# ChenWu98/cycle-diffusion

Measured on AMD Instinct MI355X. Metric: images/sec, SD-v1.4 512px CycleDiffusion 100+100 steps, 1/2/4/8 MI355X, higher is better.
Workload: dtype fp16; 1 GPU; C2: Stable-Diffusion-v1.4-shaped U-Net + KL-f8 VAE, 512x512, custom_steps=99 white_box_steps=100 eta=0.1 skip 0, 1 trial, encoder scale 1, decoder CFG 3; batch_per_gpu=4, global_batch=4, parallelism=dp1, steps_per_launch_set=5, launch_set_cap=16, launch_sets_in_flight_per_gpu=1, images_in_flight_per_gpu=20, distributed=single process, weights=synthetic(seed=0)

## Files before the change

cycle-diffusion_amd/_ffi.py:

```python
import ctypes as C
import os

import numpy as np

_HERE = os.path.dirname(os.path.abspath(__file__))
LIB_PATH = os.path.join(_HERE, "lib", "libcyclediff.so")

CD_NET_UNET_OPENAI, CD_NET_UNET_HO, CD_NET_VAE_KL, CD_NET_CLIP_TEXT, CD_NET_BERT_XTR = 1, 2, 3, 4, 5
CD_NET_OCLIP_TEXT, CD_NET_OCLIP_VISION, CD_NET_INCEPTION_FID = 6, 7, 8
CD_SCHED_DDIM, CD_SCHED_DDPM = 0, 1
CD_PREC_16, CD_PREC_F32, CD_PREC_F32X3 = 0, 1, 2
CD_MASK_QSAMPLE, CD_MASK_ENCODER = 0, 1
MASK_SOURCES = {"q_sample": CD_MASK_QSAMPLE, "encoder": CD_MASK_ENCODER}
ACT_NONE, ACT_SILU, ACT_GELU, ACT_GEGLU, ACT_QGELU, ACT_RELU = 0, 1, 2, 3, 4, 5


class NetDesc(C.Structure):
    _fields_ = [
        ("kind", C.c_int), ("image_size", C.c_int), ("in_channels", C.c_int), ("out_channels", C.c_int),
        ("model_channels", C.c_int), ("num_res_blocks", C.c_int),
        ("n_mult", C.c_int), ("channel_mult", C.c_int * 8),
        ("n_attn", C.c_int), ("attn", C.c_int * 8),
        ("num_heads", C.c_int), ("num_head_channels", C.c_int),
        ("use_spatial_transformer", C.c_int), ("context_dim", C.c_int), ("transformer_depth", C.c_int),
# ... 46 lines not shown
    "cd_cycle_translate_masked": [_VP, _I, _I, _VP, _VP, _VP, _F, _VP, _VP, _F, _VP, _I, _I, _I, _I, _VP, _VP, _VP, _U64, _I,
                                  _VP, _VP, _I, _I, _VP, _VP, _U64, _VP, _VP],
    "cd_cycle_translate_ctrl": [_VP, _I, _I, _VP, _VP, _VP, _F, _VP, _VP, _F, _VP, _I, _I, _I, _I, _VP, _VP, _VP, _U64, _I,
                                _VP, _VP, _I, _I, _VP, _VP, _U64, _VP, _VP, _VP, _I, _I, _VP, _VP],
    "cd_pix_refine": [_VP, _I, _I, _VP, _I, _I, _VP, _VP, _U64],
    "cd_op_pack_conv_weight": [_VP, _VP, _I, _I, _I, _I, _I, C.POINTER(_VP), C.POINTER(_I), C.POINTER(_I)],
    "cd_op_free": [_VP, _VP],
    "cd_op_conv2d": [_VP, _VP, _I, _VP, _I, _I, _I, _I, _VP, _I, _I, _I, _I, _I, _I, _I, _VP, _VP, _VP, _I, _I, _VP],
    "cd_op_conv2d_16": [_VP, _VP, _I, _VP, _I, _I, _I, _I, _VP, _I, _I, _I, _I, _I, _I, _I, _VP, _VP, _VP, _I, _I, _VP,
                        _VP],
    "cd_op_last_gemm_config": [_VP] + [C.POINTER(_I)] * 5,
    "cd_op_up_phase_reorder": [_VP, _VP, _I, _I, _I, _I, _VP],
    "cd_op_groupnorm": [_VP, _VP, _I, _I, _I, _I, _I, _F, _VP, _VP, _VP, _I, _VP],
    "cd_op_groupnorm_ex": [_VP, _VP, _I, _I, _VP, _I, _I, _I, _I, _I, _F, _VP, _VP, _VP, _I, _I, _VP, _VP, _I, _VP],
    "cd_op_layernorm": [_VP, _VP, _I, _I, _VP, _VP, _F, _VP],
    "cd_op_attention": [_VP, _VP, _VP, _VP, _I, _I, _I, _I, _I, _F, _I, _VP],
    "cd_op_cross_attention_ctrl": [_VP, _VP, _VP, _VP, _VP, _VP, _VP, _VP, _VP, _I, _I, _I, _I, _I, _I, _I, _I, _F, _VP],
    "cd_op_softmax_rows": [_VP, _VP, _I64, _I, _VP],
    "cd_op_timestep_embedding": [_VP, _VP, _I, _I, _I, _VP],
    "cd_op_sched_step": [_VP, _I, _I, _VP, _VP, _VP, _VP, _I, _F, _VP, _VP, _I, _I, _I, _I, _VP],
    "cd_op_sched_step_masked": [_VP, _I, _VP, _VP, _VP, _I, _F, _VP, _VP, _VP, _I, _I, _F, _F, _VP, _I, _I, _I, _I, _VP, _I],
    "cd_op_bench_conv": [_VP, _I, _I, _I, _I, _I, _I, _I, _I, _I, _I, _I, _I, C.POINTER(C.c_float)],
    "cd_op_bench_mfma_sustained": [_VP, _I, C.POINTER(C.c_float), C.POINTER(C.c_float)],
    "cd_op_probe": [_VP, _I, _VP, _VP, _SZ],
}
_RESTYPES = {"cd_last_error": C.c_char_p}

_lib = None


# ... 45 lines not shown
```

cycle-diffusion_amd/csrc/capi.hip:

```cpp
#include <stdlib.h>
#include <string.h>
#include <unistd.h>

#include <algorithm>

#include "engine.h"

using namespace cd;

struct StepPacer {
  static constexpr int kAhead = 2, kRing = kAhead + 1;
  hipEvent_t ev[kRing] = {nullptr, nullptr, nullptr};
  long n = 0;
  bool enabled = true;
  void init() {
    const char* e = getenv("CYCLEDIFF_HOST_PACING");
    enabled = !(e && e[0] == '0');
    for (auto& x : ev) HIP_CHECK(hipEventCreateWithFlags(&x, hipEventBlockingSync | hipEventDisableTiming));
  }
  static void sleep_until_done(hipEvent_t e) {
    for (;;) {
      const hipError_t q = hipEventQuery(e);
      if (q == hipSuccess) return;
      if (q != hipErrorNotReady) HIP_CHECK(q);
// ... 1087 lines not shown

int cd_op_layernorm(cd_handle h, const float* x, int rows, int C, const float* gamma, const float* beta,
                    float eps, float* y) {
  CD_API_BEGIN
  enter_engine(h);
  CD_CHECK(h && x && y, "bad argument");
  ArenaScope arena_scope(h->arena);
  bf16_t* a = (bf16_t*)h->arena.alloc((size_t)rows * C * 2);
  bf16_t* o = (bf16_t*)h->arena.alloc((size_t)rows * C * 2);
  launch_nchw_to_nhwc(h->st, x, a, rows, C, 1, C, 1.f, 0.f, 0);
  launch_layernorm(h->st, a, C, o, C, rows, C, gamma, beta, eps);
  launch_nhwc_to_nchw(h->st, o, 0, C, y, rows, C, 1, 1.f, 0.f);
  CD_API_END
}

int cd_op_attention(cd_handle h, const float* q, const float* k, const float* v, int B, int H, int Tq,
                    int Tk, int D, float scale, int use_transpose_kernel, float* o) {
  CD_API_BEGIN
  enter_engine(h);
  CD_CHECK(h && q && k && v && o, "bad argument");
  ArenaScope arena_scope(h->arena);
  const int C = H * D, Tpad = round_up(Tk, 64);
  bf16_t* qb = (bf16_t*)h->arena.alloc((size_t)B * Tq * C * 2);
  bf16_t* kb = (bf16_t*)h->arena.alloc((size_t)B * Tk * C * 2);
  bf16_t* vb = (bf16_t*)h->arena.alloc((size_t)B * Tk * C * 2);
  bf16_t* ob = (bf16_t*)h->arena.alloc((size_t)B * Tq * C * 2);
  launch_nchw_to_nhwc(h->st, q, qb, B * Tq, C, 1, C, 1.f, 0.f, 0);
  launch_nchw_to_nhwc(h->st, k, kb, B * Tk, C, 1, C, 1.f, 0.f, 0);
  launch_nchw_to_nhwc(h->st, v, vb, B * Tk, C, 1, C, 1.f, 0.f, 0);
  AttnParams p;
// ... 297 lines not shown
```

cycle-diffusion_amd/csrc/conv_gemm.hip:

```cpp
#include <stdio.h>
#include <stdlib.h>
#include <string.h>

#include <algorithm>
#include <map>
#include <mutex>
#include <string>

#include "common.h"
#include "kernels.h"

namespace cd {

namespace gemm_detail {

#ifndef CD_EPI_STORE_AUX
#define CD_EPI_STORE_AUX 0
#endif
#ifndef CD_EPI_RESID_AUX
#define CD_EPI_RESID_AUX 0
#endif

typedef const __attribute__((address_space(1))) void* gptr_t;
typedef __attribute__((address_space(3))) void* lptr_t;
// ... 1170 lines not shown
void launch_conv_gemm(hipStream_t st, const ConvGemmParams& p) {
  const int Ctot = p.C0 + p.C1;
  CD_CHECK(p.C0 % 32 == 0 && p.C1 % 32 == 0, "conv_gemm: channels must be multiples of 32 (C0=%d C1=%d)", p.C0, p.C1);
  CD_CHECK(p.Ktot == p.KH * p.KW * Ctot, "conv_gemm: Ktot mismatch");
  CD_CHECK(p.zeros != nullptr, "conv_gemm: zero page missing");
  CD_CHECK(p.M > 0 && p.N > 0, "conv_gemm: empty problem");
  CD_CHECK(((uintptr_t)p.src0 & 15) == 0 && ((uintptr_t)p.wgt & 15) == 0, "conv_gemm: 16-B alignment");
  CD_CHECK((p.ld0 % 8) == 0 && (p.src1 == nullptr || (p.ld1 % 8) == 0), "conv_gemm: ld must be a multiple of 8");
  if (p.act == ACT_GEGLU) CD_CHECK(p.N % 64 == 0, "GEGLU needs packed N %% 64 == 0");
  if (p.up_phase)
    CD_CHECK(p.KH == 2 && p.KW == 2 && p.stride == 1 && !p.up && !p.src1 && p.nbatch == 1 && p.Hout == p.Hs && p.Wout == p.Ws &&
                 (p.Hs * p.Ws) % 256 == 0 && p.M == 4 * p.B * p.Hs * p.Ws && p.w_ps > 0 && p.Hin == p.Hs && p.Win == p.Ws,
             "conv_gemm: phase form of an x2 conv on %d x %d", p.Hs, p.Ws);
  bool k64 = (p.C0 % 64 == 0) && (p.C1 % 64 == 0);
  if (p.ln_fold) CD_CHECK(p.tile == kLinStreamTile, "conv_gemm: a LayerNorm-folded layer runs on lin_stream only");
  int id = p.tile ? p.tile : tuned_config(st, p, k64);
  if (id & (1 << 16)) k64 = false;
  ConvGemmParams pk = p;
  id &= 0xffff;
  if ((id >> 8) > 1) pk.splitk = id >> 8;
  id &= 0xff;
  if (pk.splitk > 1 && !pk.sk_scratch) { pk.sk_scratch = g_conv_splitk.scratch; pk.sk_flags = g_conv_splitk.flags; }
  pk.probe = g_conv_probe;
  static const int korder_env = [] { const char* e = getenv("CYCLEDIFF_KORDER"); return e ? atoi(e) : -1; }();
  if (korder_env >= 0) pk.korder = korder_env;
  static const int tg_env = [] { const char* e = getenv("CYCLEDIFF_TILE_GROUP"); return e ? atoi(e) : 8; }();
  static const int tg_min_n = [] { const char* e = getenv("CYCLEDIFF_TILE_GROUP_MIN_N"); return e ? atoi(e) : 2048; }();
  if (tg_env > 0 && p.N >= tg_min_n && p.nbatch == 1) pk.tile_group = tg_env;
#ifdef CD_PROBE
  if (const char* e = getenv("CYCLEDIFF_PROBE_DBG")) pk.dbg = atoi(e);
// ... 117 lines not shown
```

cycle-diffusion_amd/csrc/engine.h:

```cpp
#pragma once
#include <map>
#include <memory>
#include <string>
#include <vector>

#include "common.h"
#include "kernels.h"
#include "../../include/cyclediff.h"

namespace cd {

class Arena {
 public:
  ~Arena();
  void init(size_t bytes);
  void* alloc(size_t bytes);
  size_t mark() const { return off_; }
  void release(size_t m) { off_ = m; }
  void reset() { off_ = 0; }
  size_t capacity() const { return cap_; }
  size_t high_water() const { return high_; }
 private:
  char* base_ = nullptr;
  size_t cap_ = 0, off_ = 0, high_ = 0;
// ... 93 lines not shown

struct ConvOpts {
  int stride = 1;
  int pad = 1;
  bool asym = false;
  bool up = false;
  const float* rowvec = nullptr; int rowvec_ld = 0; int rows_per_vec = 1;
  const Act* resid = nullptr;
  int act = ACT_NONE;
  float alpha = 1.f;
  bool out_f32 = false;
  void* out = nullptr;
  int out_ld = 0;
  bool ln_fold = false;
  float ln_eps = 1e-5f;
  bool raw_geglu = false;
  bool want_stats = false;
  float* out_stats = nullptr;
  int tile = 0;
};
Act attention_flash_f32_fwd(Ctx& c, const float* q, int ldq, const float* k, int ldk, int64_t k_bs, const float* v, int ldv,
                            int64_t v_bs, int B, int H, int Tq, int Tk, int D, float scale, int Himg, int Wimg, bool q_log2);
Act geglu_f32_fwd(Ctx& c, const Act& h);
Act split_rows_f32_fwd(Ctx& c, const Act& x, const Act* x2 = nullptr);
Act alloc_act(Ctx& c, int B, int H, int W, int C, bool with_stats = false);
Act conv_fwd(Ctx& c, const ConvW& w, const Act& x, const Act* x2, const ConvOpts& o);
bool conv_up_phase_taken(const Ctx& c, const ConvW& w, const Act& x, const Act* x2, const ConvOpts& o);
bool conv_ln_fold_available(const Ctx& c, const ConvW& w, int64_t rows);

struct GNW { float* g = nullptr; float* b = nullptr; int C = 0; float eps = 1e-5f; };
Act groupnorm_fwd(Ctx& c, const GNW& w, const Act& x, const Act* x2, bool silu, const float* film = nullptr,
                  int film_ld = 0);
struct LNW { float* g = nullptr; float* b = nullptr; int C = 0; };
Act layernorm_fwd(Ctx& c, const LNW& w, const Act& x);

Act avgpool2_fwd(Ctx& c, const Act& x);
Act upsample2_fwd(Ctx& c, const Act& x);
Act attention_f32_fwd(Ctx& c, const Act& qk, const Act& v, int H, int D, float scale, const float* obias);

Act attention_fwd(Ctx& c, const bf16_t* q, int ldq, const bf16_t* k, int ldk, const bf16_t* v, int ldv, int B,
                  int H, int Tq, int Tk, int D, float scale, int Himg, int Wimg, bool q_log2 = false);
Act attention_vt_fwd(Ctx& c, const bf16_t* q, int ldq, const bf16_t* k, int ldk, const bf16_t* vt, int B,
                     int H, int Tq, int Tk, int Tpad, int D, float scale, int Himg, int Wimg, bool q_log2 = false);
// ... 80 lines not shown
```

cycle-diffusion_amd/csrc/engine.hip:

```cpp
#include <stdlib.h>

#include "engine.h"

#include <string.h>

namespace cd {

Arena::~Arena() { if (base_) (void)hipFree(base_); }
void Arena::init(size_t bytes) {
  if (base_) { (void)hipFree(base_); base_ = nullptr; }
  HIP_CHECK(hipMalloc((void**)&base_, bytes));
  cap_ = bytes; off_ = 0; high_ = 0;
}
void* Arena::alloc(size_t bytes) {
  size_t a = (off_ + 255) & ~(size_t)255;
  CD_CHECK(a + bytes <= cap_, "workspace arena exhausted: need %zu more bytes (capacity %zu); "
           "create the engine with a larger workspace", a + bytes - cap_, cap_);
  off_ = a + bytes;
  if (off_ > high_) high_ = off_;
  return base_ + a;
}

ParamStore::~ParamStore() {
  for (void* p : allocs_) (void)hipFree(p);
// ... 309 lines not shown
  p.B = x.B; p.Hs = x.H; p.Ws = x.W; p.up = o.up ? 1 : 0;
  p.Hin = o.up ? x.H * 2 : x.H; p.Win = o.up ? x.W * 2 : x.W;
  p.KH = w.KH; p.KW = w.KW; p.stride = o.stride;
  if (o.asym) { p.pad_t = 0; p.pad_l = 0; p.Hout = (p.Hin + 1 - w.KH) / o.stride + 1; p.Wout = (p.Win + 1 - w.KW) / o.stride + 1; }
  else {
    p.pad_t = o.pad; p.pad_l = o.pad;
    p.Hout = (p.Hin + 2 * o.pad - w.KH) / o.stride + 1;
    p.Wout = (p.Win + 2 * o.pad - w.KW) / o.stride + 1;
  }
  p.M = x.B * p.Hout * p.Wout;
  p.wgt = w.w; p.wgt_frag = w.wfrag; p.Ktot = w.Ktot(); p.N = w.N;
  p.alpha = o.alpha; p.bias = w.b;
  p.rowvec = o.rowvec; p.rowvec_ld = o.rowvec_ld; p.rows_per_vec = o.rows_per_vec;
  const bool fuse_geglu = w.geglu && !o.raw_geglu;
  p.act = fuse_geglu ? ACT_GEGLU : o.act;
  const int Nout = fuse_geglu ? w.N / 2 : w.N;
  Act y; y.B = x.B; y.H = p.Hout; y.W = p.Wout; y.C = Nout; y.f32 = c.f32;
  if (o.out) { y.p = (bf16_t*)o.out; y.ld = o.out_ld; }
  else {
    y.ld = Nout;
    y.p = (bf16_t*)c.arena->alloc((size_t)p.M * Nout * ((o.out_f32 || c.f32) ? 4 : 2));
  }
  if (o.resid) {
    CD_CHECK(o.resid->rows() == p.M && o.resid->C == Nout, "conv: residual shape mismatch");
    p.resid = o.resid->p; p.resid_ld = o.resid->ld;
  }
  p.out = y.p; p.out_ld = y.ld; p.out_f32 = o.out_f32 ? 1 : 0;
  p.zeros = c.zeros; p.tile = o.tile;
  if (o.ln_fold) { p.ln_fold = 1; p.ln_eps = o.ln_eps; p.tile = kLinStreamTile; }
  if (c.f32) {
    p.out_f32 = 1;
    launch_conv_gemm_f32(c.st, p);
    return y;
  }
  if (!w.geglu && !o.out_f32 && ((p.Hout * p.Wout) % 32) == 0) {
    if (o.out && o.out_stats) y.stats_buf = o.out_stats;
    else if (!o.out && o.want_stats)
      y.stats_buf = (float*)c.arena->alloc((size_t)(p.M / 32) * 2 * Nout * sizeof(float));
    p.stats = y.stats_buf;
    y.stats = y.stats_buf;
  }
  launch_conv_gemm(c.st, p);
  return y;
}

bool conv_ln_fold_available(const Ctx& c, const ConvW& w, int64_t rows) {
  static const bool on = [] { const char* e = getenv("CYCLEDIFF_LN_FOLD"); return !(e && e[0] == '0'); }();
  static const int64_t min_rows = [] { const char* e = getenv("CYCLEDIFF_LN_FOLD_MIN_ROWS"); return e ? atoll(e) : 32768ll; }();
  return on && !c.f32 && w.wfrag && w.KH == 1 && w.KW == 1 && w.Cpad == 320 && rows >= min_rows && rows % 32 == 0 &&
         w.N % 64 == 0 && w.N <= 2560;
}

Act groupnorm_fwd(Ctx& c, const GNW& w, const Act& x, const Act* x2, bool silu, const float* film,
                  int film_ld) {
  GroupNormParams p;
  p.x = x.p; p.C0 = x.C; p.ld0 = x.ld;
  if (x2) { p.x1 = x2->p; p.C1 = x2->C; p.ld1 = x2->ld; }
  const int C = p.C0 + p.C1;
  CD_CHECK(C == w.C, "groupnorm: channels %d != weight %d", C, w.C);
  p.B = x.B; p.HW = x.H * x.W; p.G = 32; p.eps = w.eps; p.gamma = w.g; p.beta = w.b;
  p.film = film; p.film_ld = film_ld; p.silu = silu ? 1 : 0;
  Act y = alloc_act(c, x.B, x.H, x.W, C);
  p.y = y.p;
  if (c.f32) {
    CD_CHECK(x.f32 && (!x2 || x2->f32) && !x.split && (!x2 || !x2->split), "groupnorm: operand precision");
// ... 133 lines not shown
```

cycle-diffusion_amd/csrc/kernels.h:

```cpp
#pragma once
#include <map>
#include <string>
#include <vector>

#include "common.h"

namespace cd {

struct StepCoef {
  float sa, s1a, sap, dirc, sigma, r, t_mask;
  int t;
};
enum { SCHED_DDIM = 0, SCHED_DDPM = 1 };

struct EpsHat {
  const float* p = nullptr;
  int64_t sb = 0, sc = 0, sp = 0;
  int cfg = 0;
  float g = 1.f;
  const float* gvec = nullptr;
};

struct StepGeom {
  int B = 0, C = 0, HW = 0;
// ... 67 lines not shown
  float alpha = 1.0f;
  const float* bias = nullptr;
  const float* rowvec = nullptr;
  int rowvec_ld = 0, rows_per_vec = 1;
  const bf16_t* resid = nullptr;
  int resid_ld = 0;
  int resid_f32 = 0;
  int act = ACT_NONE;
  void* out = nullptr;
  int out_ld = 0;
  int out_f32 = 0;
  float* stats = nullptr;
  const bf16_t* zeros = nullptr;
  int ln_fold = 0;
  float ln_eps = 1e-5f;
  int tile = 0;
  float prof_flop_scale = 1.f;
  int splitk = 0;
  float* sk_scratch = nullptr;
  int* sk_flags = nullptr;
  unsigned long long* probe = nullptr;
  int korder = 1;
  int tile_group = 0;
  int dephase_ticks = 0;
  int num_cus = 256;
  int dbg = 0;
  int up_phase = 0;
  int w_ps = 0;
};
constexpr int kProbeWords = 48;
// ... 17 lines not shown
GemmLaunchInfo conv_gemm_last_launch();
void launch_up_phase_weights(hipStream_t st, const bf16_t* w, bf16_t* out, int Npad, int Cpad);
int conv_gemm_num_configs();
const char* conv_gemm_config_name(int id);

struct LinStreamParams {
  const bf16_t* a = nullptr; int lda = 0;
  const bf16_t* wfrag = nullptr;
  const float* bias = nullptr;
  const bf16_t* resid = nullptr; int ldr = 0;
  bf16_t* out = nullptr; int ldo = 0;
  float* stats = nullptr;
  int M = 0, N = 0;
  float ln_eps = 1e-5f;
  int geglu_direct = 0;
};
constexpr int kLinStreamTile = 30;
bool lin_stream_supports(const ConvGemmParams& p);
void launch_lin_stream(hipStream_t st, const ConvGemmParams& p);
void launch_fold_ln(hipStream_t st, const bf16_t* w, int ldw, const float* gamma, const float* beta, const float* bias,
                    bf16_t* w_out, float* bias_out, int N, int Kc);
void launch_pack_wfrag(hipStream_t st, const bf16_t* w, int ldw, bf16_t* out, int N);

struct KernelProfiler {
  bool enabled = false;
  std::vector<hipEvent_t> events;
  std::vector<double> flops;
  std::vector<std::string> labels;
  int used = 0;
  bool verbose = false;
// ... 136 lines not shown
```

cycle-diffusion_amd/csrc/lin_stream.hip:

```cpp
#include <stdlib.h>

#include <mutex>

#include "common.h"
#include "kernels.h"

namespace cd {
namespace lin_detail {

typedef __attribute__((address_space(3))) void* lptr_t;
typedef __attribute__((ext_vector_type(4))) unsigned int u32x4;

constexpr int K = 320, NKS = K / 16, KSH = NKS / 2;
constexpr int WPIECE = 2 * KSH * 1024, WSLOTS = 3;
constexpr int APIECE = 128 * 128, ASLOTS = 3;
constexpr int NAP = 10;
constexpr int ST_LD = 36, ST_BYTES = 32 * ST_LD * 4;
constexpr int BIAS_MAX = 2560;
constexpr int OFF_A = WSLOTS * WPIECE, OFF_ST = OFF_A + ASLOTS * APIECE, OFF_BIAS = OFF_ST + 8 * ST_BYTES;
constexpr int LDS_BYTES = OFF_BIAS + BIAS_MAX * 4;
static_assert(LDS_BYTES <= 160 * 1024, "LDS");
constexpr unsigned kNoLoad = 0x80000000u;
constexpr int kGegluDirectDefault = 1;

// ... 31 lines not shown
#pragma unroll
  for (int i = 0; i < 4; ++i) {
    const h2 v = {(_Float16)__builtin_amdgcn_fmed3f(f[2 * i], -65504.0f, 65504.0f),
                  (_Float16)__builtin_amdgcn_fmed3f(f[2 * i + 1], -65504.0f, 65504.0f)};
    w[i] = __builtin_bit_cast(uint32_t, v);
  }
  return make_uint4(w[0], w[1], w[2], w[3]);
#else
  return pack8(f);
#endif
}
__device__ __forceinline__ void touch4(u32x4& a, u32x4& b, u32x4& c, u32x4& d) {
  asm volatile("" : "+v"(a), "+v"(b), "+v"(c), "+v"(d)::"memory");
}

template <int ACT, bool RESID, bool STATS, bool LNF = false>
__global__ __launch_bounds__(512, 2) void k_lin_stream(LinStreamParams p) {
#if defined(__HIP_DEVICE_COMPILE__)
  constexpr bool GEGLU = (ACT == ACT_GEGLU);
  static_assert(!(GEGLU && (RESID || STATS)), "GEGLU has neither residual nor statistics");
  extern __shared__ __attribute__((aligned(16))) char smem[];
  char* wring = smem;
  char* aring = smem + OFF_A;
  const int tid = threadIdx.x, lane = tid & 63;
  const int wave = __builtin_amdgcn_readfirstlane(tid >> 6);
  float* stage = (float*)(smem + OFF_ST + wave * ST_BYTES);
  float* bias_s = (float*)(smem + OFF_BIAS);
  const int mi = lane & 31, half = lane >> 5;
  const bool w_issuer = wave < 4;
  const int wq = wave & 3;

  const int NT = p.N >> 6;
  const int I = 2 * NT;
  const int nstrips = (p.M + 255) >> 8;
  const int G = gridDim.x;
// ... 159 lines not shown
        const int soff = ((row0 + 16 * ps) * p.ldr + t * 64 + nb * 32) * 2;
        asm volatile("buffer_load_dwordx4 %0, %1, %2, %3 offen"
                     : "=v"(rres[nb * 2 + ps]) : "v"(r_lane), "s"(rs_r), "s"(soff) : "memory");
      }
    seq += 4;
    rmark = seq;
  };
  issue_resid((int)blockIdx.x * 256, 0);

  int gi = 0;
  int wslot = 0;
  for (int ord = 0; ord < my_count; ++ord) {
    const int row0 = ((int)blockIdx.x + ord * G) * 256;
    const bool has_next = ord + 1 < my_count;
    const bool rows_ok = row0 + wave * 32 < p.M;
    for (int t = 0; t < NT; ++t) {
#pragma unroll
      for (int r = 0; r < 16; ++r) { acc[0][r] = 0.f; acc[1][r] = 0.f; }
#pragma unroll
      for (int kh = 0; kh < 2; ++kh) {
        const int i = 2 * t + kh;
        if (w_issuer) wait_vmcnt_le(seq - wm0);
        const bool due = a_due(gi);
        if (due && !w_issuer) wait_vmcnt_le(seq - am0);
        asm volatile("s_waitcnt lgkmcnt(0)\n\ts_barrier" ::: "memory");
        if (w_issuer) {
          const int nxt = i + 2;
          const int slot2 = wslot == 0 ? 2 : wslot - 1;
          issue_w(nxt < I ? nxt : nxt - I, nxt < I || has_next, slot2);
          seq += 5;
          wm0 = wm1; wm1 = seq;
// ... 29 lines not shown
          }
        }
        if (due) take_a(ce_j, ce_slot);
        wslot = wslot == 2 ? 0 : wslot + 1;
        ++gi;
      }
      if (RESID && rows_ok) {
        wait_vmcnt_le(seq - rmark);
        touch4(rres[0], rres[1], rres[2], rres[3]);
      }
      float vv[2][8];
      int l2 = lane;
      asm volatile("" : "+v"(l2));
      const int prow = l2 >> 2, pcol = (l2 & 3) * 8, mi2 = l2 & 31, half2 = l2 >> 5;
      const unsigned o_lane = (unsigned)(((wave * 32 + prow) * p.ldo + pcol) * 2);
      if (GEGLU && p.geglu_direct) {
        const unsigned od_lane = (unsigned)(((wave * 32 + mi2) * p.ldo + 4 * half2) * 2);
#pragma unroll
        for (int q = 0; q < 4; ++q) {
          const float* bp = bias_s + t * 64 + 8 * q + 4 * half2;
          const f32x4 bv = *(const f32x4*)bp, bg = *(const f32x4*)(bp + 32);
          float val[4], gate[4], o4[4];
#pragma unroll
          for (int j = 0; j < 4; ++j) { val[j] = acc[0][4 * q + j] + bv[j]; gate[j] = acc[1][4 * q + j] + bg[j]; }
          mul_gelu4(val, gate, o4);
          if (rows_ok) {
            typedef __attribute__((ext_vector_type(2))) unsigned int u32x2;
            const u32x2 o = {pack2(o4[0], o4[1]), pack2(o4[2], o4[3])};
            __builtin_amdgcn_raw_buffer_store_b64(o, rs_o, od_lane, (row0 * p.ldo + t * 32 + 8 * q) * 2, 0);
          }
          __builtin_amdgcn_sched_barrier(0);
// ... 93 lines not shown
__global__ void k_fold_ln(const bf16_t* __restrict__ w, int ldw, const float* __restrict__ gamma,
                          const float* __restrict__ beta, const float* __restrict__ bias, bf16_t* __restrict__ w_out,
                          float* __restrict__ bias_out, int N, int Kc) {
  const int n = blockIdx.x * (blockDim.x >> 6) + (threadIdx.x >> 6), lane = threadIdx.x & 63;
  if (n >= N) return;
  float acc = 0.f;
  for (int k = lane; k < Kc; k += 64) {
    const float x = bf2f(w[(int64_t)n * ldw + k]);
    acc = __builtin_fmaf(x, beta[k], acc);
    w_out[(int64_t)n * ldw + k] = f2bf(x * gamma[k]);
  }
  acc = wave_allsum(acc);
  if (lane == 0) bias_out[n] = (bias ? bias[n] : 0.f) + acc;
}

template <int ACT, bool RESID, bool STATS, bool LNF = false>
void launch_variant(hipStream_t st, const LinStreamParams& p, int grid) {
  static PerDeviceOnce attr_once;
  auto kern = k_lin_stream<ACT, RESID, STATS, LNF>;
  attr_once([&]() {
    HIP_CHECK(hipFuncSetAttribute((const void*)kern, hipFuncAttributeMaxDynamicSharedMemorySize, LDS_BYTES));
  });
  hipLaunchKernelGGL(kern, dim3(grid), dim3(512), LDS_BYTES, st, p);
}

}

bool lin_stream_supports(const ConvGemmParams& p) {
  if (p.KH != 1 || p.KW != 1 || p.stride != 1 || p.up || p.src1 || p.C1 != 0) return false;
  if (p.Ktot != lin_detail::K || p.C0 != lin_detail::K || p.nbatch != 1 || p.out_f32 || p.rowvec) return false;
  if (p.alpha != 1.0f || p.splitk > 1 || !p.wgt_frag) return false;
  if (p.N % 64 != 0 || p.N > lin_detail::BIAS_MAX || p.N < 320) return false;
  if (p.act != ACT_NONE && p.act != ACT_GEGLU) return false;
  if (p.act == ACT_GEGLU && (p.resid || p.stats)) return false;
// ... 15 lines not shown
  p.stats = c.stats; p.M = c.M; p.N = c.N;
  static std::atomic<int> ncu_of[64];
  int dev = 0;
  HIP_CHECK(hipGetDevice(&dev));
  int ncu = ncu_of[dev & 63].load(std::memory_order_relaxed);
  if (!ncu) {
    hipDeviceProp_t prop;
    HIP_CHECK(hipGetDeviceProperties(&prop, dev));
    ncu = prop.multiProcessorCount > 0 ? prop.multiProcessorCount : 256;
    ncu_of[dev & 63].store(ncu, std::memory_order_relaxed);
  }
  const int nstrips = (p.M + 255) / 256;
  const int grid = nstrips < ncu ? nstrips : ncu;
  static const int geglu_direct = [] { const char* e = getenv("CYCLEDIFF_GEGLU_DIRECT"); return e && e[0] ? atoi(e) : kGegluDirectDefault; }();
  p.geglu_direct = geglu_direct;
  if (c.ln_fold) {
    p.ln_eps = c.ln_eps;
    CD_CHECK(!c.resid && !c.stats, "lin_stream: a LayerNorm-folded layer has neither residual nor statistics");
    if (c.act == ACT_GEGLU) launch_variant<ACT_GEGLU, false, false, true>(st, p, grid);
    else launch_variant<ACT_NONE, false, false, true>(st, p, grid);
    return;
  }
  if (c.act == ACT_GEGLU) launch_variant<ACT_GEGLU, false, false>(st, p, grid);
  else if (c.resid && c.stats) launch_variant<ACT_NONE, true, true>(st, p, grid);
  else if (c.resid) launch_variant<ACT_NONE, true, false>(st, p, grid);
  else if (c.stats) launch_variant<ACT_NONE, false, true>(st, p, grid);
  else launch_variant<ACT_NONE, false, false>(st, p, grid);
}

void launch_fold_ln(hipStream_t st, const bf16_t* w, int ldw, const float* gamma, const float* beta, const float* bias,
                    bf16_t* w_out, float* bias_out, int N, int Kc) {
  hipLaunchKernelGGL(lin_detail::k_fold_ln, dim3((N + 3) / 4), dim3(256), 0, st, w, ldw, gamma, beta, bias, w_out,
                     bias_out, N, Kc);
// ... 12 lines not shown
```

cycle-diffusion_amd/csrc/unet_openai.hip:

```cpp
#include <limits.h>

#include <algorithm>

#include "engine.h"

namespace cd {

namespace {

struct ResW {
  int cin = 0, cout = 0;
  bool up = false, down = false, film = false;
  GNW gn1, gn2;
  ConvW *conv1 = nullptr, *conv2 = nullptr, *skip = nullptr;
  int emb_off = 0;
};

struct STW {
  int C = 0, heads = 0, dh = 0, ctx = 0;
  GNW norm;
  ConvW *proj_in = nullptr, *proj_out = nullptr;
  LNW ln1, ln2, ln3;
  ConvW *qkv1 = nullptr, *qk1 = nullptr, *v1 = nullptr, *o1 = nullptr;
  ConvW *q2 = nullptr, *k2 = nullptr, *v2 = nullptr, *o2 = nullptr;
  ConvW *ff1 = nullptr, *ff2 = nullptr;
  ConvW *q2_ln = nullptr, *ff1_ln = nullptr;
  bf16_t* k2c = nullptr;
  bf16_t* v2c = nullptr;
};

struct ABW {
  int C = 0, heads = 0, dh = 0;
  GNW norm;
  ConvW *qk = nullptr, *v = nullptr, *proj = nullptr;
  float* vbias = nullptr;
};

struct Layer {
  enum Kind { CONV_IN, RES, ST, AB, DOWN_CONV, UP_CONV } kind;
  int idx = 0;
  ConvW* conv = nullptr;
// ... 95 lines not shown
    s.qkv1 = params.new_conv(3 * C, C, 1, 1, false);
    params.conv_rows(tb + ".attn1.to_q.weight", {C, C}, s.qkv1, 0, C, 0, C, 0, qscale);
    params.conv_rows(tb + ".attn1.to_k.weight", {C, C}, s.qkv1, C, C, 0, C, 0);
    params.conv_rows(tb + ".attn1.to_v.weight", {C, C}, s.qkv1, 2 * C, C, 0, C, 0);
  }
  s.o1 = make_conv(params, tb + ".attn1.to_out.0", C, C, 1, true, false, 2);
  s.q2 = make_conv(params, tb + ".attn2.to_q", C, C, 1, false, false, 2, qscale);
  s.k2 = make_conv(params, tb + ".attn2.to_k", C, s.ctx, 1, false, false, 2);
  s.v2 = make_conv(params, tb + ".attn2.to_v", C, s.ctx, 1, false, false, 2);
  s.o2 = make_conv(params, tb + ".attn2.to_out.0", C, C, 1, true, false, 2);
  s.ff1 = make_conv(params, tb + ".ff.net.0.proj", 8 * C, C, 1, true, true, 2);
  s.ff2 = make_conv(params, tb + ".ff.net.2", C, 4 * C, 1, true, false, 2);
  if (s.q2->wfrag) {
    s.q2_ln = params.new_conv(C, C, 1, 1, true);
    s.ff1_ln = params.new_conv(8 * C, C, 1, 1, true, true);
  }
  st_.push_back(s);
  return (int)st_.size() - 1;
}

int UNetOpenAI::add_ab(const std::string& pfx, int C, int heads) {
  ABW a; a.C = C; a.heads = heads; a.dh = C / heads;
  a.norm = make_gn(params, pfx + ".norm", C, 1e-5f);
  const int ch = a.dh;
  a.qk = params.new_conv(2 * C, C, 1, 1, true);
  a.v = params.new_conv(C, C, 1, 1, false);
  a.vbias = params.new_vec(C);
  const std::string wn = pfx + ".qkv.weight", bn = pfx + ".qkv.bias";
  params.conv_rows(wn, {3 * C, C, 1}, a.qk, 0, C, 0, ch, 3 * ch);
  params.conv_rows(wn, {3 * C, C, 1}, a.qk, C, C, ch, ch, 3 * ch);
// ... 329 lines not shown
}

void UNetOpenAI::st_core16(Ctx& c, STW& s, const Act& x_in, const Act& x, Act& out, int b0, int dup_tail) {
  const bool dup = dup_tail > 0;
  int B = x_in.B;
  const int T = x_in.H * x_in.W, C = s.C;
  const size_t mk = c.arena->mark();
  ConvOpts p0; p0.pad = 0;
  const float scale = 1.0f / sqrtf((float)s.dh);
  const bf16_t* k2c = s.k2c + (int64_t)b0 * ctx_L_ * C;
  const bf16_t* v2c = s.v2c + (int64_t)b0 * ctx_L_ * C;
  Act n = groupnorm_fwd(c, s.norm, x_in, nullptr, false);
  Act h = conv_fwd(c, *s.proj_in, n, nullptr, p0);
  {
    const size_t m2 = c.arena->mark();
    Act n1 = layernorm_fwd(c, s.ln1, h);
    Act a;
    if (s.qkv1) {
      Act qkv = conv_fwd(c, *s.qkv1, n1, nullptr, p0);
      a = attention_fwd(c, qkv.p, qkv.ld, qkv.p + C, qkv.ld, qkv.p + 2 * C, qkv.ld, B, s.heads, T, T, s.dh, scale,
                        x.H, x.W, true);
    } else {
      Act qk = conv_fwd(c, *s.qk1, n1, nullptr, p0);
      const int Tpad = round_up(T, 64);
      bf16_t* vt = (bf16_t*)c.arena->alloc((size_t)B * C * Tpad * 2);
      if (Tpad != T) HIP_CHECK(hipMemsetAsync(vt, 0, (size_t)B * C * Tpad * 2, c.st));
      vt_gemm(c, *s.v1, n1.p, n1.ld, B, T, Tpad, vt);
      a = attention_vt_fwd(c, qk.p, qk.ld, qk.p + C, qk.ld, vt, B, s.heads, T, T, Tpad, s.dh, scale, x.H, x.W,
                           true);
    }
    ConvOpts o; o.pad = 0; o.resid = &h; o.out = h.p; o.out_ld = h.ld;
    conv_fwd(c, *s.o1, a, nullptr, o);
    c.arena->release(m2);
  }
  if (dup) {
    Act h2 = alloc_act(c, B + dup_tail, x_in.H, x_in.W, C);
    dup_rows(c, h.p, h2.p, (int64_t)B * T, (int64_t)dup_tail * T, C);
    h = h2;
    B += dup_tail;
  }
  {
    const size_t m2 = c.arena->mark();
// ... 107 lines not shown
}

void UNetOpenAI::refresh_ln_folds(Ctx& c) {
  if (folded_version_ == params.version) return;
  for (const Block& b : out_blocks_)
    for (const Layer& l : b.layers)
      if (l.kind == Layer::UP_CONV) params.refresh_up_phase(c.st, l.conv);
  for (STW& s : st_) {
    if (!s.q2_ln) continue;
    struct { const ConvW* src; ConvW* dst; const LNW* ln; } jobs[2] = {{s.q2, s.q2_ln, &s.ln2}, {s.ff1, s.ff1_ln, &s.ln3}};
    for (auto& j : jobs) {
      launch_fold_ln(c.st, j.src->w, j.src->Ktot(), j.ln->g, j.ln->b, j.src->b, j.dst->w, j.dst->b, j.src->Npad,
                     j.src->Cpad);
      launch_pack_wfrag(c.st, j.dst->w, j.dst->Ktot(), j.dst->wfrag, j.dst->Npad);
    }
  }
  folded_version_ = params.version;
}

void UNetOpenAI::forward(Ctx& c, const UNetIO& io) {
  const size_t mk0 = c.arena->mark();
  c.f32 = f32; c.x3 = x3;
  refresh_ln_folds(c);
  CD_CHECK(!io.ctrl || (!f32 && io.ctrl->va.size() == st_.size()), "U-Net: cross-attention control on a network it was not built for");
  ctrl_ = io.ctrl;
  const int B = io.B, R = image_size;
  const int tB = io.t_shared ? 1 : B;
  float* sinu = (float*)c.arena->alloc((size_t)tB * mc_ * 4);
  float* e1 = (float*)c.arena->alloc((size_t)tB * hidden_ * 4);
  float* emb = (float*)c.arena->alloc((size_t)tB * hidden_ * 4);
// ... 42 lines not shown
  h = run_block(c, mid_, h, nullptr, proj, proj_ld, io.t_shared);
  for (const Block& b : out_blocks_) {
    Act skip = hs.back(); hs.pop_back();
    h = run_block(c, b, h, &skip, proj, proj_ld, io.t_shared);
  }
  Act hn = groupnorm_fwd(c, out_norm_, h, nullptr, true);
  ConvOpts oo; oo.out_f32 = true; oo.out = io.out; oo.out_ld = io.out_ld;
  conv_fwd(c, *out_conv_, hn, nullptr, oo);
  c.arena->release(mk0);
  c.f32 = false; c.x3 = false;
  ctrl_ = nullptr;
}

}

std::unique_ptr<UNet> make_unet_openai(const cd_net_desc& d) { return std::unique_ptr<UNet>(new UNetOpenAI(d)); }

}
```

include/cyclediff.h:

```cpp
#ifndef CYCLEDIFF_H
#define CYCLEDIFF_H
#include <stddef.h>
#include <stdint.h>

#ifdef __cplusplus
extern "C" {
#endif

typedef struct cd_engine* cd_handle;

enum { CD_NET_UNET_OPENAI = 1, CD_NET_UNET_HO = 2, CD_NET_VAE_KL = 3, CD_NET_CLIP_TEXT = 4, CD_NET_BERT_XTR = 5,
       CD_NET_OCLIP_TEXT = 6, CD_NET_OCLIP_VISION = 7, CD_NET_INCEPTION_FID = 8 };
enum { CD_SCHED_DDIM = 0, CD_SCHED_DDPM = 1 };
enum { CD_PREC_16 = 0, CD_PREC_F32 = 1, CD_PREC_F32X3 = 2 };
enum { CD_MASK_QSAMPLE = 0, CD_MASK_ENCODER = 1 };

typedef struct cd_net_desc {
  int kind;
  int image_size;
  int in_channels, out_channels;
  int model_channels;
  int num_res_blocks;
  int n_mult;  int channel_mult[8];
  int n_attn;  int attn[8];
// ... 100 lines not shown
                 const void* packed_w, int N, int KH, int KW, int stride, int pad, int asym_pad, int up,
                 const float* bias, const float* rowvec, const float* resid, int act, int tile, float* y);
int cd_op_conv2d_16(cd_handle h, const float* x0, int C0, const float* x1, int C1, int B, int H, int W,
                    const void* packed_w, int N, int KH, int KW, int stride, int pad, int asym_pad, int up,
                    const float* bias, const float* rowvec, const float* resid, int act, int tile, float* y,
                    float* stats);
int cd_op_last_gemm_config(cd_handle h, int* tile_id, int* bk, int* splitk, int* chm, int* tile_group);
int cd_op_up_phase_reorder(cd_handle h, const float* x, int B, int C, int H, int W, float* y);
int cd_op_groupnorm(cd_handle h, const float* x, int B, int C, int H, int W, int G, float eps,
                    const float* gamma, const float* beta, const float* film, int silu, float* y);
int cd_op_groupnorm_ex(cd_handle h, const float* x0, int C0, int pad0, const float* x1, int C1, int pad1, int B, int H,
                       int W, float eps, const float* gamma, const float* beta, const float* film, int film_ld, int silu,
                       const float* stats0, const float* stats1, int precision, void* y);
int cd_op_layernorm(cd_handle h, const float* x, int rows, int C, const float* gamma, const float* beta,
                    float eps, float* y);
int cd_op_attention(cd_handle h, const float* q, const float* k, const float* v, int B, int H, int Tq,
                    int Tk, int D, float scale, int use_transpose_kernel, float* o);
int cd_op_cross_attention_ctrl(cd_handle h, const float* q_own, const float* q_src, const float* k_own, const float* k_src,
                               const float* v_own, const float* mapper, const float* alpha, const float* weight, int B,
                               int B_src, int B_ctrl, int H, int Tq, int L, int L_buf, int D, float scale, float* o);
int cd_op_softmax_rows(cd_handle h, const float* s, int64_t rows, int cols, float* p);
int cd_op_timestep_embedding(cd_handle h, const float* t, int B, int dim, int mode, float* out);
int cd_op_sched_step(cd_handle h, int mode, int sched_kind, const cd_step_coef* coef_host, const float* x0,
                     float* xt, const float* eps_hat, int cfg, float guidance, const float* noise,
                     const float* eps_in, int is_last, int B, int C, int HW, float* z_slot);
int cd_op_sched_step_masked(cd_handle h, int mode, const cd_step_coef* coef_host, float* x, const float* eps_hat, int cfg,
                            float guidance, const float* eps_in, const float* mask, const float* src, int B_mask,
                            int mask_source, float qa, float qb, const float* mask_noise, int blend, int B, int C, int HW,
                            void* xin16_out, int cfg_dup);
int cd_op_bench_conv(cd_handle h, int B, int H, int W, int C0, int C1, int N, int k, int stride, int up,
// ... 9 lines not shown
```

Before: 3.542 images/s.

## Fuse LayerNorm, Q|K projection and transposed V projection into one streaming GEMM

For self-attention in the spatial transformer, the LayerNorm is folded into a combined q|k|v weight, and a single lin_stream launch writes Q|K row-major and V transposed straight into the attention's V^T buffer. This replaces a separate layernorm kernel, the QK GEMM and the vt_gemm, which removes the normalized activation round trip and two launches. It applies only when T is a multiple of 256, C pads to 320 and there are enough rows, so other blocks keep the old path. It adds scattered 16-bit buffer stores for the transposed V columns and a test entry point with fold modes.

```diff
diff --git a/cycle-diffusion_amd/_ffi.py b/cycle-diffusion_amd/_ffi.py
--- a/cycle-diffusion_amd/_ffi.py
+++ b/cycle-diffusion_amd/_ffi.py
@@ -84,6 +84,7 @@
     "cd_op_groupnorm": [_VP, _VP, _I, _I, _I, _I, _I, _F, _VP, _VP, _VP, _I, _VP],
     "cd_op_groupnorm_ex": [_VP, _VP, _I, _I, _VP, _I, _I, _I, _I, _I, _F, _VP, _VP, _VP, _I, _I, _VP, _VP, _I, _VP],
     "cd_op_layernorm": [_VP, _VP, _I, _I, _VP, _VP, _F, _VP],
+    "cd_op_self_attn_qkv": [_VP, _VP, _I, _I, _I, _I, _VP, _VP, _VP, _VP, _VP, _I, _I, _VP, _VP, C.POINTER(_I)],
     "cd_op_attention": [_VP, _VP, _VP, _VP, _I, _I, _I, _I, _I, _F, _I, _VP],
     "cd_op_cross_attention_ctrl": [_VP, _VP, _VP, _VP, _VP, _VP, _VP, _VP, _VP, _I, _I, _I, _I, _I, _I, _I, _I, _F, _VP],
     "cd_op_softmax_rows": [_VP, _VP, _I64, _I, _VP],
diff --git a/cycle-diffusion_amd/csrc/capi.hip b/cycle-diffusion_amd/csrc/capi.hip
--- a/cycle-diffusion_amd/csrc/capi.hip
+++ b/cycle-diffusion_amd/csrc/capi.hip
@@ -1125,6 +1125,63 @@
   CD_API_END
 }
 
+int cd_op_self_attn_qkv(cd_handle h, const float* x, int B, int T, int C, int heads, const float* ln_gamma,
+                        const float* ln_beta, const float* wq_host, const float* wk_host, const float* wv_host, int mode,
+                        int guard, float* qk, float* vt, int* fused) {
+  CD_API_BEGIN
+  enter_engine(h);
+  CD_CHECK(h && x && ln_gamma && ln_beta && wq_host && wk_host && wv_host && qk && vt, "bad argument");
+  CD_CHECK(B > 0 && T > 0 && C > 0 && C % 64 == 0 && heads > 0 && C % heads == 0 && mode >= 0 && mode <= 3, "bad argument");
+  CD_CHECK(guard >= 0 && guard % 64 == 0, "bad argument (guard: a multiple of 64 elements)");
+  ArenaScope arena_scope(h->arena);
+  Ctx c = h->ctx();
+  static int counter = 0;
+  const std::string pfx = "op.qkv." + std::to_string(counter++);
+  const float qscale = 1.44269504088896340736f / sqrtf((float)(C / heads));
+  ParamStore& ps = h->op_params;
+  ConvW* wqk = ps.new_conv(2 * C, C, 1, 1, false);
+  ConvW* wv = ps.new_conv(C, C, 1, 1, false);
+  ps.conv_rows(pfx + ".q", {C, C}, wqk, 0, C, 0, C, 0, qscale);
+  ps.conv_rows(pfx + ".k", {C, C}, wqk, C, C, 0, C, 0);
+  ps.conv_weight(pfx + ".v", wv, 2);
+  const int64_t shape[2] = {C, C};
+  ps.load(h->st, pfx + ".q", wq_host, 2, shape);
+  ps.load(h->st, pfx + ".k", wk_host, 2, shape);
+  ps.load(h->st, pfx + ".v", wv_host, 2, shape);
+  LNW ln; ln.g = const_cast<float*>(ln_gamma); ln.b = const_cast<float*>(ln_beta); ln.C = C;
+  ConvW* wqkv_ln = nullptr;
+  if (wqk->wfrag && mode != 0) {
+    wqkv_ln = ps.new_conv(3 * C, C, 1, 1, true);
+    build_qkv_fold(h->st, *wqk, *wv, ln, *wqkv_ln);
+  }
+  Act a = alloc_act(c, B, T, 1, C);
+  launch_nchw_to_nhwc(h->st, x, a.p, B * T, C, 1, C, 1.f, 0.f, 0);
+  const int Tpad = round_up(T, 64);
+  const size_t nvt = (size_t)B * C * Tpad;
+  bf16_t* vbuf = (bf16_t*)h->arena.alloc((nvt + 2 * (size_t)guard) * 2);
+  HIP_CHECK(hipMemsetAsync(vbuf, 0x7b, (nvt + 2 * (size_t)guard) * 2, h->st));
+  bf16_t* vt16 = vbuf + guard;
+  int tp = 0;
+  bool fold = false;
+  Act q;
+  if (mode == 3) {
+    CD_CHECK(wqk->wfrag && (int64_t)B * T % 32 == 0, "mode 3 needs the streaming kernel's shapes (C = 320, rows %% 32 == 0)");
+    ConvW* wqk_ln = ps.new_conv(2 * C, C, 1, 1, true);
+    launch_fold_ln(h->st, wqk->w, wqk->Ktot(), ln.g, ln.b, nullptr, wqk_ln->w, wqk_ln->b, wqk->N, wqk->Cpad);
+    launch_pack_wfrag(h->st, wqk_ln->w, wqk_ln->Ktot(), wqk_ln->wfrag, wqk_ln->Npad);
+    ConvOpts pl; pl.pad = 0; pl.ln_fold = true;
+    q = conv_fwd(c, *wqk_ln, a, nullptr, pl);
+    (void)self_attn_qkv_fwd(c, ln, *wqk, *wv, nullptr, a, B, T, &vt16, &tp);
+  } else {
+    q = self_attn_qkv_fwd(c, ln, *wqk, *wv, wqkv_ln, a, B, T, &vt16, &tp, mode == 2, &fold);
+  }
+  CD_CHECK(tp == Tpad && q.ld == 2 * C, "self-attention projections: layout");
+  if (fused) *fused = fold ? 1 : 0;
+  launch_nhwc_to_nchw(h->st, q.p, 0, q.ld, qk, B * T, 2 * C, 1, 1.f, 0.f);
+  launch_nhwc_to_nchw(h->st, vbuf, 0, 64, vt, (int)((nvt + 2 * (size_t)guard) / 64), 64, 1, 1.f, 0.f);
+  CD_API_END
+}
+
 int cd_op_attention(cd_handle h, const float* q, const float* k, const float* v, int B, int H, int Tq,
                     int Tk, int D, float scale, int use_transpose_kernel, float* o) {
   CD_API_BEGIN
diff --git a/cycle-diffusion_amd/csrc/conv_gemm.hip b/cycle-diffusion_amd/csrc/conv_gemm.hip
--- a/cycle-diffusion_amd/csrc/conv_gemm.hip
+++ b/cycle-diffusion_amd/csrc/conv_gemm.hip
@@ -1208,6 +1208,7 @@
              "conv_gemm: phase form of an x2 conv on %d x %d", p.Hs, p.Ws);
   bool k64 = (p.C0 % 64 == 0) && (p.C1 % 64 == 0);
   if (p.ln_fold) CD_CHECK(p.tile == kLinStreamTile, "conv_gemm: a LayerNorm-folded layer runs on lin_stream only");
+  if (p.vt) CD_CHECK(p.ln_fold, "conv_gemm: a V-transposed output is written by the LayerNorm-folded lin_stream launch only");
   int id = p.tile ? p.tile : tuned_config(st, p, k64);
   if (id & (1 << 16)) k64 = false;
   ConvGemmParams pk = p;
diff --git a/cycle-diffusion_amd/csrc/engine.h b/cycle-diffusion_amd/csrc/engine.h
--- a/cycle-diffusion_amd/csrc/engine.h
+++ b/cycle-diffusion_amd/csrc/engine.h
@@ -131,6 +131,8 @@
   int out_ld = 0;
   bool ln_fold = false;
   float ln_eps = 1e-5f;
+  bf16_t* vt = nullptr;
+  int n_split = 0, vt_tpad = 0;
   bool raw_geglu = false;
   bool want_stats = false;
   float* out_stats = nullptr;
@@ -144,6 +146,12 @@
 Act conv_fwd(Ctx& c, const ConvW& w, const Act& x, const Act* x2, const ConvOpts& o);
 bool conv_up_phase_taken(const Ctx& c, const ConvW& w, const Act& x, const Act* x2, const ConvOpts& o);
 bool conv_ln_fold_available(const Ctx& c, const ConvW& w, int64_t rows);
+bool qkv_fold_available(const Ctx& c, const ConvW& w, int B, int T, bool force = false);
+
+struct LNW;
+Act self_attn_qkv_fwd(Ctx& c, const LNW& ln, const ConvW& qk, const ConvW& v, const ConvW* qkv_ln, const Act& h, int B,
+                      int T, bf16_t** vt, int* Tpad, bool force = false, bool* fused = nullptr);
+void build_qkv_fold(hipStream_t st, const ConvW& qk, const ConvW& v, const LNW& ln, ConvW& dst);
 
 struct GNW { float* g = nullptr; float* b = nullptr; int C = 0; float eps = 1e-5f; };
 Act groupnorm_fwd(Ctx& c, const GNW& w, const Act& x, const Act* x2, bool silu, const float* film = nullptr,
diff --git a/cycle-diffusion_amd/csrc/engine.hip b/cycle-diffusion_amd/csrc/engine.hip
--- a/cycle-diffusion_amd/csrc/engine.hip
+++ b/cycle-diffusion_amd/csrc/engine.hip
@@ -347,7 +347,8 @@
   p.rowvec = o.rowvec; p.rowvec_ld = o.rowvec_ld; p.rows_per_vec = o.rows_per_vec;
   const bool fuse_geglu = w.geglu && !o.raw_geglu;
   p.act = fuse_geglu ? ACT_GEGLU : o.act;
-  const int Nout = fuse_geglu ? w.N / 2 : w.N;
+  CD_CHECK(!o.vt || (o.ln_fold && !fuse_geglu && o.n_split > 0 && o.n_split < w.N), "conv: V-transposed output columns");
+  const int Nout = o.vt ? o.n_split : (fuse_geglu ? w.N / 2 : w.N);
   Act y; y.B = x.B; y.H = p.Hout; y.W = p.Wout; y.C = Nout; y.f32 = c.f32;
   if (o.out) { y.p = (bf16_t*)o.out; y.ld = o.out_ld; }
   else {
@@ -361,6 +362,7 @@
   p.out = y.p; p.out_ld = y.ld; p.out_f32 = o.out_f32 ? 1 : 0;
   p.zeros = c.zeros; p.tile = o.tile;
   if (o.ln_fold) { p.ln_fold = 1; p.ln_eps = o.ln_eps; p.tile = kLinStreamTile; }
+  if (o.vt) { p.vt = o.vt; p.vt_split = o.n_split; p.vt_T = p.Hout * p.Wout; p.vt_tpad = o.vt_tpad; }
   if (c.f32) {
     p.out_f32 = 1;
     launch_conv_gemm_f32(c.st, p);
@@ -382,6 +384,15 @@
   static const int64_t min_rows = [] { const char* e = getenv("CYCLEDIFF_LN_FOLD_MIN_ROWS"); return e ? atoll(e) : 32768ll; }();
   return on && !c.f32 && w.wfrag && w.KH == 1 && w.KW == 1 && w.Cpad == 320 && rows >= min_rows && rows % 32 == 0 &&
          w.N % 64 == 0 && w.N <= 2560;
+}
+
+constexpr bool kQkvFoldDefault = true;
+bool qkv_fold_available(const Ctx& c, const ConvW& w, int B, int T, bool force) {
+  const char* e = getenv("CYCLEDIFF_QKV_FOLD");
+  if (e && e[0] ? e[0] == '0' : !kQkvFoldDefault) return false;
+  if (T % 256 != 0 || w.N % 3 != 0 || (w.N / 3 * 2) % 64 != 0) return false;
+  if (force) return !c.f32 && w.wfrag && w.KH == 1 && w.KW == 1 && w.Cpad == 320 && w.N % 64 == 0 && w.N <= 2560;
+  return conv_ln_fold_available(c, w, (int64_t)B * T);
 }
 
 Act groupnorm_fwd(Ctx& c, const GNW& w, const Act& x, const Act* x2, bool silu, const float* film,
diff --git a/cycle-diffusion_amd/csrc/kernels.h b/cycle-diffusion_amd/csrc/kernels.h
--- a/cycle-diffusion_amd/csrc/kernels.h
+++ b/cycle-diffusion_amd/csrc/kernels.h
@@ -105,6 +105,8 @@
   const bf16_t* zeros = nullptr;
   int ln_fold = 0;
   float ln_eps = 1e-5f;
+  bf16_t* vt = nullptr;
+  int vt_split = 0, vt_T = 0, vt_tpad = 0;
   int tile = 0;
   float prof_flop_scale = 1.f;
   int splitk = 0;
@@ -152,6 +154,8 @@
   int M = 0, N = 0;
   float ln_eps = 1e-5f;
   int geglu_direct = 0;
+  bf16_t* vt = nullptr;
+  int n_split = 0, T = 0;
 };
 constexpr int kLinStreamTile = 30;
 bool lin_stream_supports(const ConvGemmParams& p);
diff --git a/cycle-diffusion_amd/csrc/lin_stream.hip b/cycle-diffusion_amd/csrc/lin_stream.hip
--- a/cycle-diffusion_amd/csrc/lin_stream.hip
+++ b/cycle-diffusion_amd/csrc/lin_stream.hip
@@ -69,11 +69,12 @@
   asm volatile("" : "+v"(a), "+v"(b), "+v"(c), "+v"(d)::"memory");
 }
 
-template <int ACT, bool RESID, bool STATS, bool LNF = false>
+template <int ACT, bool RESID, bool STATS, bool LNF = false, bool VT = false>
 __global__ __launch_bounds__(512, 2) void k_lin_stream(LinStreamParams p) {
 #if defined(__HIP_DEVICE_COMPILE__)
   constexpr bool GEGLU = (ACT == ACT_GEGLU);
   static_assert(!(GEGLU && (RESID || STATS)), "GEGLU has neither residual nor statistics");
+  static_assert(!VT || (ACT == ACT_NONE && !RESID && !STATS), "the V-transposed variant is a plain projection");
   extern __shared__ __attribute__((aligned(16))) char smem[];
   char* wring = smem;
   char* aring = smem + OFF_A;
@@ -263,7 +264,9 @@
     const int row0 = ((int)blockIdx.x + ord * G) * 256;
     const bool has_next = ord + 1 < my_count;
     const bool rows_ok = row0 + wave * 32 < p.M;
+    const int img = VT ? row0 / p.T : 0;
     for (int t = 0; t < NT; ++t) {
+      const bool vtile = VT && t * 64 >= p.n_split;
 #pragma unroll
       for (int r = 0; r < 16; ++r) { acc[0][r] = 0.f; acc[1][r] = 0.f; }
 #pragma unroll
@@ -323,7 +326,32 @@
       asm volatile("" : "+v"(l2));
       const int prow = l2 >> 2, pcol = (l2 & 3) * 8, mi2 = l2 & 31, half2 = l2 >> 5;
       const unsigned o_lane = (unsigned)(((wave * 32 + prow) * p.ldo + pcol) * 2);
-      if (GEGLU && p.geglu_direct) {
+      if (VT && vtile) {
+        const int CV = p.N - p.n_split;
+        const __amdgpu_buffer_rsrc_t rs_v =
+            __builtin_amdgcn_make_buffer_rsrc((void*)p.vt, 0, (unsigned)((size_t)p.M * CV * 2), 0x00020000);
+        const unsigned v_lane = (unsigned)((4 * half2 * p.T + mi2) * 2);
+        const int tok0 = row0 - img * p.T + wave * 32;
+        int so = ((img * CV + t * 64 - p.n_split) * p.T + tok0) * 2;
+        const int row1 = 2 * p.T, row5 = 10 * p.T;
+#pragma unroll
+        for (int nb = 0; nb < 2; ++nb) {
+#pragma unroll
+          for (int q = 0; q < 4; ++q) {
+            const f32x4 bv = *(const f32x4*)(bias_s + t * 64 + nb * 32 + 8 * q + 4 * half2);
+            const uint32_t w01 = pack2(acc[nb][4 * q] + bv[0], acc[nb][4 * q + 1] + bv[1]);
+            const uint32_t w23 = pack2(acc[nb][4 * q + 2] + bv[2], acc[nb][4 * q + 3] + bv[3]);
+            const short v4[4] = {(short)w01, (short)(w01 >> 16), (short)w23, (short)(w23 >> 16)};
+#pragma unroll
+            for (int j = 0; j < 4; ++j) {
+              asm volatile("" : "+s"(so));
+              if (rows_ok) __builtin_amdgcn_raw_buffer_store_b16(v4[j], rs_v, v_lane, so, 0);
+              so += j < 3 ? row1 : row5;
+            }
+            __builtin_amdgcn_sched_barrier(0);
+          }
+        }
+      } else if (GEGLU && p.geglu_direct) {
         const unsigned od_lane = (unsigned)(((wave * 32 + mi2) * p.ldo + 4 * half2) * 2);
 #pragma unroll
         for (int q = 0; q < 4; ++q) {
@@ -447,10 +475,10 @@
   if (lane == 0) bias_out[n] = (bias ? bias[n] : 0.f) + acc;
 }
 
-template <int ACT, bool RESID, bool STATS, bool LNF = false>
+template <int ACT, bool RESID, bool STATS, bool LNF = false, bool VT = false>
 void launch_variant(hipStream_t st, const LinStreamParams& p, int grid) {
   static PerDeviceOnce attr_once;
-  auto kern = k_lin_stream<ACT, RESID, STATS, LNF>;
+  auto kern = k_lin_stream<ACT, RESID, STATS, LNF, VT>;
   attr_once([&]() {
     HIP_CHECK(hipFuncSetAttribute((const void*)kern, hipFuncAttributeMaxDynamicSharedMemorySize, LDS_BYTES));
   });
@@ -496,9 +524,20 @@
   const int grid = nstrips < ncu ? nstrips : ncu;
   static const int geglu_direct = [] { const char* e = getenv("CYCLEDIFF_GEGLU_DIRECT"); return e && e[0] ? atoi(e) : kGegluDirectDefault; }();
   p.geglu_direct = geglu_direct;
+  CD_CHECK(!c.vt || c.ln_fold, "lin_stream: the V-transposed output belongs to the LayerNorm-folded q | k | v projection");
   if (c.ln_fold) {
     p.ln_eps = c.ln_eps;
     CD_CHECK(!c.resid && !c.stats, "lin_stream: a LayerNorm-folded layer has neither residual nor statistics");
+    if (c.vt) {
+      CD_CHECK(c.act == ACT_NONE && c.vt_split > 0 && c.vt_split < c.N && c.vt_split % 64 == 0 && c.out_ld >= c.vt_split,
+               "lin_stream: V-transposed columns [%d, %d) of a row of %d", c.vt_split, c.N, c.out_ld);
+      CD_CHECK(c.vt_T > 0 && c.vt_T % 256 == 0 && c.M % c.vt_T == 0 && c.vt_tpad == c.vt_T,
+               "lin_stream: V-transposed output needs T %% 256 == 0 and Tpad == T (M %d T %d Tpad %d)", c.M, c.vt_T, c.vt_tpad);
+      CD_CHECK(((uintptr_t)c.vt & 7) == 0, "lin_stream: V^T alignment");
+      p.vt = c.vt; p.n_split = c.vt_split; p.T = c.vt_T;
+      launch_variant<ACT_NONE, false, false, true, true>(st, p, grid);
+      return;
+    }
     if (c.act == ACT_GEGLU) launch_variant<ACT_GEGLU, false, false, true>(st, p, grid);
     else launch_variant<ACT_NONE, false, false, true>(st, p, grid);
     return;
diff --git a/cycle-diffusion_amd/csrc/unet_openai.hip b/cycle-diffusion_amd/csrc/unet_openai.hip
--- a/cycle-diffusion_amd/csrc/unet_openai.hip
+++ b/cycle-diffusion_amd/csrc/unet_openai.hip
@@ -25,6 +25,7 @@
   ConvW *q2 = nullptr, *k2 = nullptr, *v2 = nullptr, *o2 = nullptr;
   ConvW *ff1 = nullptr, *ff2 = nullptr;
   ConvW *q2_ln = nullptr, *ff1_ln = nullptr;
+  ConvW* qkv1_ln = nullptr;
   bf16_t* k2c = nullptr;
   bf16_t* v2c = nullptr;
 };
@@ -150,6 +151,7 @@
   if (s.q2->wfrag) {
     s.q2_ln = params.new_conv(C, C, 1, 1, true);
     s.ff1_ln = params.new_conv(8 * C, C, 1, 1, true, true);
+    if (s.qk1) s.qkv1_ln = params.new_conv(3 * C, C, 1, 1, true);
   }
   st_.push_back(s);
   return (int)st_.size() - 1;
@@ -509,18 +511,16 @@
   Act h = conv_fwd(c, *s.proj_in, n, nullptr, p0);
   {
     const size_t m2 = c.arena->mark();
-    Act n1 = layernorm_fwd(c, s.ln1, h);
     Act a;
     if (s.qkv1) {
+      Act n1 = layernorm_fwd(c, s.ln1, h);
       Act qkv = conv_fwd(c, *s.qkv1, n1, nullptr, p0);
       a = attention_fwd(c, qkv.p, qkv.ld, qkv.p + C, qkv.ld, qkv.p + 2 * C, qkv.ld, B, s.heads, T, T, s.dh, scale,
                         x.H, x.W, true);
     } else {
-      Act qk = conv_fwd(c, *s.qk1, n1, nullptr, p0);
-      const int Tpad = round_up(T, 64);
-      bf16_t* vt = (bf16_t*)c.arena->alloc((size_t)B * C * Tpad * 2);
-      if (Tpad != T) HIP_CHECK(hipMemsetAsync(vt, 0, (size_t)B * C * Tpad * 2, c.st));
-      vt_gemm(c, *s.v1, n1.p, n1.ld, B, T, Tpad, vt);
+      int Tpad = 0;
+      bf16_t* vt = nullptr;
+      Act qk = self_attn_qkv_fwd(c, s.ln1, *s.qk1, *s.v1, s.qkv1_ln, h, B, T, &vt, &Tpad);
       a = attention_vt_fwd(c, qk.p, qk.ld, qk.p + C, qk.ld, vt, B, s.heads, T, T, Tpad, s.dh, scale, x.H, x.W,
                            true);
     }
@@ -658,6 +658,7 @@
                      j.src->Cpad);
       launch_pack_wfrag(c.st, j.dst->w, j.dst->Ktot(), j.dst->wfrag, j.dst->Npad);
     }
+    if (s.qkv1_ln) build_qkv_fold(c.st, *s.qk1, *s.v1, s.ln1, *s.qkv1_ln);
   }
   folded_version_ = params.version;
 }
@@ -730,6 +731,34 @@
 
 }
 
+void build_qkv_fold(hipStream_t st, const ConvW& qk, const ConvW& v, const LNW& ln, ConvW& dst) {
+  CD_CHECK(dst.wfrag && dst.b && qk.N == 2 * v.N && dst.N == 3 * v.N && qk.Ktot() == dst.Ktot() && v.Ktot() == dst.Ktot() &&
+               ln.C == dst.Cin, "q | k | v fold: shapes");
+  launch_fold_ln(st, qk.w, qk.Ktot(), ln.g, ln.b, qk.b, dst.w, dst.b, qk.N, qk.Cpad);
+  launch_fold_ln(st, v.w, v.Ktot(), ln.g, ln.b, v.b, dst.w + (int64_t)qk.N * dst.Ktot(), dst.b + qk.N, v.N, v.Cpad);
+  launch_pack_wfrag(st, dst.w, dst.Ktot(), dst.wfrag, dst.Npad);
+}
+
+Act self_attn_qkv_fwd(Ctx& c, const LNW& ln, const ConvW& qk, const ConvW& v, const ConvW* qkv_ln, const Act& h, int B,
+                      int T, bf16_t** vt_out, int* Tpad_out, bool force, bool* fused) {
+  const int C = v.N, Tpad = round_up(T, 64);
+  CD_CHECK(h.rows() == (int64_t)B * T && qk.N == 2 * C, "self-attention projections: %d x %d tokens", B, T);
+  bf16_t* vt = *vt_out ? *vt_out : (bf16_t*)c.arena->alloc((size_t)B * C * Tpad * 2);
+  *vt_out = vt; *Tpad_out = Tpad;
+  const bool fold = qkv_ln && Tpad == T && qkv_fold_available(c, *qkv_ln, B, T, force);
+  if (fused) *fused = fold;
+  if (fold) {
+    ConvOpts pl; pl.pad = 0; pl.ln_fold = true; pl.vt = vt; pl.n_split = 2 * C; pl.vt_tpad = Tpad;
+    return conv_fwd(c, *qkv_ln, h, nullptr, pl);
+  }
+  ConvOpts p0; p0.pad = 0;
+  Act n1 = layernorm_fwd(c, ln, h);
+  Act q = conv_fwd(c, qk, n1, nullptr, p0);
+  if (Tpad != T) HIP_CHECK(hipMemsetAsync(vt, 0, (size_t)B * C * Tpad * 2, c.st));
+  vt_gemm(c, v, n1.p, n1.ld, B, T, Tpad, vt);
+  return q;
+}
+
 std::unique_ptr<UNet> make_unet_openai(const cd_net_desc& d) { return std::unique_ptr<UNet>(new UNetOpenAI(d)); }
 
 }
diff --git a/include/cyclediff.h b/include/cyclediff.h
--- a/include/cyclediff.h
+++ b/include/cyclediff.h
@@ -138,6 +138,9 @@
                        const float* stats0, const float* stats1, int precision, void* y);
 int cd_op_layernorm(cd_handle h, const float* x, int rows, int C, const float* gamma, const float* beta,
                     float eps, float* y);
+int cd_op_self_attn_qkv(cd_handle h, const float* x, int B, int T, int C, int heads, const float* ln_gamma,
+                        const float* ln_beta, const float* wq_host, const float* wk_host, const float* wv_host, int mode,
+                        int guard, float* qk, float* vt, int* fused);
 int cd_op_attention(cd_handle h, const float* q, const float* k, const float* v, int B, int H, int Tq,
                     int Tk, int D, float scale, int use_transpose_kernel, float* o);
 int cd_op_cross_attention_ctrl(cd_handle h, const float* q_own, const float* q_src, const float* k_own, const float* k_src,
```

New measurement: 3.573 images/s (median of 6 runs). No clear change (+0.9%).
